# rsutormin/KmerGutsJava

Hardware: AMD Instinct MI355X
Metric: amino-acid residues/sec scanned (and hits/sec) on 1 Gbp synthetic, 1/2/4/8 MI355X (higher is better)
Workload: dtype int64; 1 GPU; 1 Gbp contig mix (0.5 kbp..1.024 Mbp, uniform ACGT) on 1 GPU, 6-frame translate + 8-mer lookup vs 1400303159-slot signature table (33.6 GB, load 0.50), -m 5 -g 200; total_bp_rank0=1000000000, contigs_rank0=6351, total_bp_all_ranks=1000000000, num_sigs=1400303159, residues_rank0=1999974596, residues_all_ranks=1999974596, hits_rank0=36744843, hits_all_ranks=36744843, calls_rank0=4, parallelism=contig shards x1, table replicated

## Files before the change

### kmergutsjava_amd/csrc/kg_host_plan.hpp

```cpp
#pragma once

namespace {


template <typename T, T V, T... Vs, typename F>
void dispatch(T x, F &&f)
{
    if constexpr (sizeof...(Vs) == 0) f(std::integral_constant<T, V>{});
    else if (x == V) f(std::integral_constant<T, V>{});
    else dispatch<T, Vs...>(x, f);
}

struct BatchPlan {
    std::vector<uint32_t> ibase;
    uint64_t nblocks = 0, windows = 0, residues = 0;
    uint64_t n_rows = 0, n_cont = 0;
    int64_t longest = 0;
};

template <bool AA>
int plan_batch(const int64_t *offsets, int64_t n_seqs, BatchPlan &b)
{
    constexpr uint32_t PER = AA ? 1 : 6;
    b.ibase.resize((size_t)n_seqs + 1);
    for (int64_t k = 0; k < n_seqs; k++) {
        int64_t L = offsets[k + 1] - offsets[k];
        if (L < 0) return fail(KG_ERR_ARG, "offsets must be non-decreasing");
        b.longest = std::max(b.longest, L);
        if (L > 0xFFFFFFF0ll) return fail(KG_ERR_LIMIT, "a single sequence longer than 2^32-16 characters");
        b.ibase[(size_t)k] = (uint32_t)b.nblocks;
        uint64_t nb;
        if (AA) {
            uint64_t nwin = L >= 9 ? (uint64_t)L - 8 : 0;
            b.windows += nwin;
            b.residues += (uint64_t)L;
            nb = (nwin + kg::kAaWinPerBlock - 1) / kg::kAaWinPerBlock;
        } else {
            uint64_t npos = L >= 24 ? (uint64_t)L - 23 : 0;
            b.windows += 2 * npos;
            for (int f = 0; f < 3; f++)
                if (L - f >= 3) b.residues += 2 * (uint64_t)((L - f) / 3);
            nb = (npos + kg::kDnaPosPerBlock - 1) / kg::kDnaPosPerBlock;
        }
        b.nblocks += nb;
        if (b.nblocks > 0x7FFFFFFFull / PER) return fail(KG_ERR_LIMIT, "batch too large: more than 2^31-1 window rows; split the batch");
    }
    b.ibase[(size_t)n_seqs] = (uint32_t)b.nblocks;
    if (b.windows > 0xFFFFFF00ull) return fail(KG_ERR_LIMIT, "batch too large: more than 2^32-256 windows; split the batch");
    b.n_rows = b.nblocks * PER;
    b.n_cont = (uint64_t)n_seqs * PER;
    return KG_OK;
}

uint64_t bucket_count(uint64_t limit, uint32_t shift) { return (limit + (1ull << shift) - 1) >> shift; }

struct PartPlan {
    bool applicable = false;
    uint32_t shift = 0, buckets = 0;
    uint32_t n_chunks = 0;
    std::vector<uint64_t> clo;
    std::vector<int64_t> cseq;
    uint64_t max_chunk = 0;
    uint32_t n_wg = 0, cap = 0;
    uint64_t n_regions = 0;
    uint32_t ovf_cap = 0;
    uint32_t gshift = 10, groups_stride = 0;
    size_t next_stride = 0;
    size_t scatter_lds = 0;
    bool use_bidx = false, part_counters = false, prog_index = false;
    uint32_t probe_grid = 0, index_grid = 0, verify_grid = 0, lowc_grid = 0, ovf_grid = 0, order_grid = 0;
    uint32_t scatter_prio = 0, index_prio = 0, verify_prio = 0, index_r = 1, probe_grab = 0;
    uint64_t list_slack = 0, ucap = 0, ccap = 0;
    uint32_t n_os = 0;
    bool early_totals = false, place_staged = false, debug = false;
};

template <bool AA>
int plan_partition(const kg_table *t, const BatchPlan &b, bool progress, bool counters_req, PartPlan &pl)
{
    constexpr uint32_t PER = AA ? 1 : 6;
    const uint64_t nblocks = b.nblocks;
    uint32_t shift = env_knob("KG_PART_SHIFT", 21u, 4u, 31u);
    const uint64_t qmax = (uint64_t)KG_MAX_ENCODED / (uint64_t)t->num_sigs + 1;
    while (shift > 4 && qmax >= (1ull << (32 - shift))) shift--;
    while (bucket_count(t->limit, shift) > (uint64_t)kg::kMaxBuckets) shift++;
    while (kg::scatter_lds_bytes<AA>((uint32_t)bucket_count(t->limit, shift)) > 160u * 1024) shift++;
    const bool fits = shift < 32 && qmax < (1ull << (32 - shift)) && nblocks <= (1ull << 23) && t->m35 != 0 &&
                      t->limit < (1ull << 32) - 64;
    const uint32_t mode = env_u32("KG_PARTITION", 2u);
    const bool worth = t->limit >= (64ull << 20) && b.windows >= (1ull << 27);
    if (!(fits && nblocks > 0 && (mode == 1 || (mode == 2 && worth)))) return KG_OK;
    pl.shift = shift;
    pl.buckets = (uint32_t)bucket_count(t->limit, shift);

    constexpr uint32_t WIN = AA ? 64u : 384u;
    uint32_t want = env_u32("KG_PART_CHUNKS", 4u);
    if (want < 1) want = 1;
    if (want > kMaxChunks) want = kMaxChunks;
    if (getenv("KG_PART_MIN_CHUNK_BLOCKS")) {
        const uint64_t min_chunk = std::max(1u, env_u32("KG_PART_MIN_CHUNK_BLOCKS", 600000u));
        while (want > 1 && nblocks / want < min_chunk) want--;
    } else {
        const uint32_t by_size = nblocks < 450000 ? 1u : std::max(2u, (uint32_t)std::lround(std::sqrt((double)nblocks / 325000.0)));
        want = std::min(want, std::max(1u, by_size));
    }
    pl.clo.push_back(0); pl.cseq.push_back(0);
    std::vector<double> cum;
    if (const char *tp = getenv("KG_PART_TAPER")) {
        double acc = 0;
        for (const char *q = tp; *q;) {
            char *endp = nullptr;
            const double v = strtod(q, &endp);
            if (endp == q) break;
            acc += v; cum.push_back(acc);
            q = *endp == ',' ? endp + 1 : endp;
        }
        if (cum.size() >= 2 && cum.size() <= kMaxChunks && acc > 0) { for (auto &x : cum) x /= acc; want = (uint32_t)cum.size(); }
        else cum.clear();
    }
    for (uint32_t c = 1; c < want; c++) {
        const uint64_t target = cum.empty() ? nblocks * c / want : (uint64_t)((double)nblocks * cum[c - 1]);
        const auto it = std::lower_bound(b.ibase.begin(), b.ibase.end(), (uint32_t)target);
        const uint64_t cut = *it;
        if (cut > pl.clo.back() && cut < nblocks) { pl.clo.push_back(cut); pl.cseq.push_back((int64_t)(it - b.ibase.begin())); }
    }
    pl.clo.push_back(nblocks); pl.cseq.push_back((int64_t)b.ibase.size() - 1);
    pl.n_chunks = (uint32_t)pl.clo.size() - 1;
    for (uint32_t c = 0; c < pl.n_chunks; c++) pl.max_chunk = std::max(pl.max_chunk, pl.clo[c + 1] - pl.clo[c]);
    const uint64_t max_chunk = pl.max_chunk;
    const uint64_t chunk_blocks = (max_chunk + kg::kScatterWaves - 1) / kg::kScatterWaves * kg::kScatterWaves;
    const double max_frac = (double)max_chunk / (double)nblocks;
    uint32_t n_wg = env_knob("KG_PART_WGS", 256u, 1u, kMaxGrid);
    if ((uint64_t)n_wg * kg::kScatterWaves > chunk_blocks) n_wg = (uint32_t)((chunk_blocks + kg::kScatterWaves - 1) / kg::kScatterWaves);
    const uint64_t blocks_per_wg = ((chunk_blocks + (uint64_t)n_wg * kg::kScatterWaves - 1) / ((uint64_t)n_wg * kg::kScatterWaves)) * kg::kScatterWaves;
    const double mean = (double)blocks_per_wg * WIN / (double)pl.buckets * (env_u32("KG_PART_SLACK", 100u) / 100.0);
    const uint64_t cap64 = ((uint64_t)(mean + 6.0 * std::sqrt(mean) + 32.0) + 15) / 16 * 16;
    if (cap64 >= (1ull << 24) || (uint64_t)pl.buckets * n_wg >= (1ull << 24)) return KG_OK;
    pl.n_wg = n_wg;
    pl.cap = (uint32_t)cap64;
    pl.n_regions = (uint64_t)pl.buckets * n_wg;
    pl.ovf_cap = env_u32("KG_PART_OVF_GROUPS", (uint32_t)std::min<uint64_t>(1u << 23, std::max<uint64_t>(65536, pl.n_regions * pl.cap / 16 / 8)));
    while (pl.gshift < 12 && ((max_chunk * PER) >> pl.gshift) + 2 > 8192) pl.gshift++;
    pl.groups_stride = (uint32_t)(((max_chunk * PER) >> pl.gshift) + 2);
    if (pl.groups_stride > kg::kMaxGroups) return fail(KG_ERR_LIMIT, "a chunk of the batch holds more than 2^26 window rows");
    pl.next_stride = std::max<size_t>((size_t)pl.buckets + 8, 256);
    pl.use_bidx = t->d_bidx != nullptr && !counters_req && env_u32("KG_BIDX", 1u) != 0;
    pl.part_counters = (counters_req || progress) && !pl.use_bidx;
    pl.prog_index = progress && pl.use_bidx;
    pl.scatter_lds = kg::scatter_lds_bytes<AA>(pl.buckets);
    pl.probe_grid = env_knob("KG_PROBE_GRID", 256u * 8u, 8u, kMaxGrid, 8u);
    pl.index_grid = env_knob("KG_INDEX_GRID", 256u * 4u, 8u, kMaxGrid, 8u);
    pl.scatter_prio = std::min(3u, env_u32("KG_SCATTER_PRIO", 1u));
    pl.index_prio = std::min(3u, env_u32("KG_INDEX_PRIO", 2u));
    pl.verify_prio = std::min(3u, env_u32("KG_VERIFY_PRIO", pl.n_chunks == 1 ? 2u : 0u));
    uint32_t index_r = env_u32("KG_INDEX_R", 0u);
    if (index_r == 0) index_r = mean * 0.7 >= 640.0 ? 1u : mean * 0.7 >= 320.0 ? 2u : 4u;
    if (index_r != 1 && index_r != 2) index_r = 4;
    while (index_r > 1 && (n_wg % index_r != 0 || kg::kIndexN % index_r != 0)) index_r /= 2;
    pl.index_r = index_r;
    pl.verify_grid = env_knob("KG_VERIFY_GRID", 256u * 2u, 1u, kMaxGrid);
    pl.lowc_grid = env_knob("KG_LOWC_GRID", 256u, 1u, kMaxGrid);
    pl.ovf_grid = env_knob("KG_OVF_GRID", 256u, 1u, kMaxGrid);
    pl.list_slack = (uint64_t)(std::max(std::max(pl.probe_grid, pl.index_grid), pl.verify_grid) + 64) * 4 * kg::kUChunk + 4096;
    pl.ucap = ((uint64_t)((double)b.windows * t->stage_ratio * max_frac) + pl.list_slack + kg::kUChunk - 1) / kg::kUChunk * kg::kUChunk;
    pl.ccap = ((uint64_t)((double)b.windows * (t->stage_ratio * 1.25 + 0.03) * max_frac) + pl.list_slack + kg::kUChunk - 1) /
              kg::kUChunk * kg::kUChunk;
    if (test_hook("KG_TEST_TINY_LISTS")) pl.ucap = pl.ccap = kg::kUChunk;
    const uint32_t grab_unit = 256u * (uint32_t)std::max(kg::kProbeN, kg::kIndexN);
    pl.probe_grab = env_knob("KG_PROBE_GRAB", pl.cap, grab_unit, 1u << 24, grab_unit);
    pl.n_os = pl.n_chunks < 2 ? 0u : std::min(env_u32("KG_ORDER_STREAMS", 0u), kMaxOrderStreams);
    pl.early_totals = pl.n_os == 0 && env_u32("KG_EARLY_TOTALS", 1u) != 0;
    pl.order_grid = env_knob("KG_ORDER_GRID", 256u * 3u, 1u, kMaxGrid);
    pl.place_staged = pl.gshift == 10 && env_u32("KG_PLACE_STAGED", 1u) != 0;
    pl.debug = getenv("KG_DEBUG") != nullptr;
    pl.applicable = true;
    return KG_OK;
}

struct DirectPlan {
    uint32_t scan_grid, stage_chunk;
    const uint32_t *d_hbits;
    uint32_t rpg;
    uint64_t stage_cap;
};

template <bool AA>
DirectPlan plan_direct(const kg_table *t, const BatchPlan &b, bool counters)
{
    DirectPlan pl;
    pl.scan_grid = env_knob("KG_SCAN_GRID", 256u * 8u, 1u, kMaxGrid);
    pl.stage_chunk = env_knob("KG_STAGE_CHUNK", 256u, 1u, 1u << 12);
    const uint32_t filter_mode = env_u32("KG_DIRECT_FILTER", 1u);
    pl.d_hbits = (counters || filter_mode == 0 || (filter_mode == 1 && t->limit <= (4ull << 20))) ? nullptr : t->d_hbits;
    pl.rpg = AA ? 1u : env_u32("KG_SCAN_RPG", pl.d_hbits ? 6u : 3u);
    if (pl.rpg != 1 && pl.rpg != 2 && pl.rpg != 3 && pl.rpg != 6) pl.rpg = 3;
    pl.stage_cap = (uint64_t)((double)b.windows * t->stage_ratio) + 4096 + (uint64_t)pl.scan_grid * kg::kWavesPerWG * pl.stage_chunk;
    if (pl.stage_cap > 0xFFFFFF00ull) pl.stage_cap = 0xFFFFFF00ull;
    if (test_hook("KG_TEST_TINY_LISTS")) pl.stage_cap = 256;
    return pl;
}

struct AggPlan {
    uint32_t pshift;
    bool pieces_on;
    uint32_t agg_pairs;
};

AggPlan plan_aggregate()
{
    AggPlan pl;
    pl.pshift = std::min(20u, std::max(6u, env_u32("KG_AGG_BLOCK_SHIFT", 9u)));
    pl.pieces_on = env_u32("KG_AGG_PIECES", 1u) != 0;
    pl.agg_pairs = env_u32("KG_AGG_PAIRS", 1u);
    return pl;
}

}
```

### kmergutsjava_amd/csrc/kg_host_scan.hpp

```cpp
#pragma once

namespace {

struct ScanCtx {
    kg_table *t;
    kg_result *res;
    Scratch &sc;
    const BatchPlan &b;
    const uint8_t *d_seq, *h_seq;
    const int64_t *offsets;
    int64_t n_seqs;
    bool progress, counters;
    bool seq_uploaded;
    uint64_t n_hits = 0;
    int64_t *d_off = nullptr;
    uint32_t *d_ibase = nullptr;
    kg::BlockDesc *d_blocks = nullptr;
    uint32_t *d_counts = nullptr, *d_offs = nullptr, *d_bsb = nullptr;
    uint64_t *d_partial = nullptr, *d_totals = nullptr;
    kg::Progress *d_prog = nullptr;
};

int upload_seq(const ScanCtx &cx, int64_t a, int64_t b)
{
// ... 114 lines not shown
    size_t cused_stride = 0, candused_stride = 0;
    kg_hit *d_ulist = nullptr, *d_sortA = nullptr, *d_sortB = nullptr;
    uint32_t *d_cused = nullptr, *d_candused = nullptr;
    kg::CandRec *d_cand = nullptr;
};

struct ChunkView {
    uint32_t c, lo, nb;
    uint64_t *ent, *ovf_ent;
    uint32_t *fill, *next, *ovfc, *ovf_bucket;
    kg_hit *ulist, *sortA, *sortB;
    uint32_t *cused, *candused;
    kg::CandRec *cand;
    unsigned long long *ucur, *ccur;
    uint64_t *base, *ctot;
    uint32_t *ghist, *gbase, *gcur1, *gcur2, *gtile;
};

ChunkView chunk_view(const PartPlan &pl, const PartBuffers &pb, uint32_t c)
{
    ChunkView v;
    v.c = c; v.lo = (uint32_t)pl.clo[c]; v.nb = (uint32_t)(pl.clo[c + 1] - pl.clo[c]);
    v.ent = pb.d_ent + (uint64_t)c * pl.n_regions * pl.cap;
    v.fill = pb.d_fill + (uint64_t)c * pl.n_regions;
    v.next = pb.d_next + (size_t)c * pl.next_stride;
    v.ovfc = pb.d_ovfc + kOvfWords * c; v.ovf_bucket = pb.d_ovf_bucket + (size_t)c * pl.ovf_cap;
    v.ovf_ent = pb.d_ovf_ent + (size_t)c * pl.ovf_cap * kg::kGroup;
    v.ulist = pb.d_ulist + (uint64_t)c * pb.ucap;
    v.cused = pb.d_cused + c * pb.cused_stride; v.candused = pb.d_candused + c * pb.candused_stride;
    v.cand = pb.d_cand + (uint64_t)c * pb.ccap;
    v.ucur = (unsigned long long *)(pb.d_pc + kPcUcur + c); v.ccur = (unsigned long long *)(pb.d_pc + kPcCcur + c);
    v.base = pb.d_pc + kPcBase + c; v.ctot = pb.d_pc + kPcCtot + c;
    v.ghist = pb.d_ghist + (size_t)c * pl.groups_stride; v.gbase = pb.d_gbase + (size_t)c * (pl.groups_stride + 1);
    v.gcur1 = pb.d_gcur1 + (size_t)c * (kg::kHDigits + 1); v.gcur2 = pb.d_gcur2 + (size_t)c * pl.groups_stride;
    v.gtile = pb.d_gtile + (size_t)c * (kg::kHDigits + 1);
    v.sortA = pb.d_sortA + (uint64_t)c * pb.ucap; v.sortB = pb.d_sortB + (uint64_t)c * pb.ucap;
    return v;
}

int scatter_variant_of(const ScanCtx &cx)
{
    return cx.t->limit >= (uint64_t)cx.t->num_sigs ? 0 : cx.d_prog ? 2 : 1;
}
template <typename F>
void scatter_variant(int variant, F &&f)
{
    if (variant == 0) f(std::false_type{}, std::false_type{});
    else if (variant == 1) f(std::true_type{}, std::false_type{});
    else f(std::true_type{}, std::true_type{});
}

int upload_scatter_cold(const ScanCtx &cx, const PartPlan &pl, const PartBuffers &pb)
{
    kg_table *t = cx.t;
    kg::ScatterCold h[kMaxChunks] = {};
    for (uint32_t c = 0; c < pl.n_chunks; c++) {
        uint32_t *ovfc = pb.d_ovfc + kOvfWords * c;
        h[c].ovf_cursor = ovfc; h[c].ovf_bucket = pb.d_ovf_bucket + (size_t)c * pl.ovf_cap;
        h[c].ovf_ent = pb.d_ovf_ent + (size_t)c * pl.ovf_cap * kg::kGroup;
        h[c].lowc_cursor = ovfc + kOvfLowc; h[c].lowc_blocks = pb.d_lowc + pl.clo[c];
        h[c].ctr = (unsigned long long *)(cx.d_totals + kTotValid); h[c].prog = cx.d_prog;
        h[c].ovf_cap = pl.ovf_cap;
    }
    if (!t->d_cold) HIP_TRY(hipMalloc((void **)&t->d_cold, sizeof h));
    else if (!memcmp(h, t->h_cold, sizeof h)) return KG_OK;
    memcpy(t->h_cold, h, sizeof h);
    HIP_TRY(hipMemcpyAsync(t->d_cold, t->h_cold, sizeof h, hipMemcpyHostToDevice, t->stream));
    return KG_OK;
}

template <bool AA>
int chunk_passes(const ScanCtx &cx, const PartPlan &pl, const PartBuffers &pb, const ChunkView &v)
{
    kg_table *t = cx.t;
    kg::Progress *d_prog = cx.d_prog;
    unsigned long long *d_ctr = (unsigned long long *)(cx.d_totals + kTotValid);
    const hipStream_t s2 = t->stream2, s3 = t->stream3;
    uint32_t *lowc_cursor = v.ovfc + kOvfLowc, *lowc = pb.d_lowc + v.lo;
    const uint32_t limit32 = (uint32_t)std::min<uint64_t>(t->limit, 0xFFFFFFFFull);
    scatter_variant(scatter_variant_of(cx), [&](auto is_short, auto prog) {
        constexpr bool SHORT = decltype(is_short)::value, PROG = decltype(prog)::value;
        hipLaunchKernelGGL((kg::part_scatter_kernel<AA, SHORT, PROG>), dim3(pl.n_wg), dim3(kg::kWave * kg::kScatterWaves), pl.scatter_lds,
                           t->stream, cx.d_seq, cx.d_blocks, v.lo, v.nb, limit32, (uint32_t)t->num_sigs, t->m35, pl.shift, pl.buckets, pl.cap,
                           v.ent, v.fill, t->d_cold + v.c, pl.scatter_prio);
    });
    HIP_TRY(hipEventRecord(t->pev[kPevChunk + 2 * v.c], t->stream));
    HIP_TRY(hipStreamWaitEvent(s2, t->pev[kPevChunk + 2 * v.c], 0));
    hipLaunchKernelGGL((kg::lowc_blocks_kernel<AA>), dim3(pl.lowc_grid), dim3(64 * kg::kLowcWaves), 0, s2, cx.d_seq, cx.d_blocks, lowc_cursor, lowc,
                       t->limit, (uint32_t)t->num_sigs, t->m35, pl.shift, pl.n_wg, pl.cap, v.ent, v.fill, v.ovfc, pl.ovf_cap,
                       v.ovf_bucket, v.ovf_ent, d_ctr, d_prog);
    if (pl.use_bidx) {
        const uint32_t tail_start = (uint32_t)std::min<uint64_t>(t->tail_start, 0xFFFFFFFFull);
        dispatch<int, 1, 2, 4>((int)pl.index_r, [&](auto r) {
            dispatch<bool, true, false>(t->bidx_exact, [&](auto exact) {
                dispatch<bool, true, false>(pl.prog_index, [&](auto prog) {
                    constexpr int R = decltype(r)::value;
                    constexpr bool EXACT = decltype(exact)::value, PROG = decltype(prog)::value;
                    hipLaunchKernelGGL((kg::bucket_index_kernel<kg::kIndexN, R, EXACT, PROG>), dim3(pl.index_grid), dim3(256), 0, s2,
                                       t->d_bidx, tail_start, v.ent, v.fill, pl.n_wg, pl.cap, pl.buckets, pl.shift, pl.probe_grab, v.next,
                                       v.cand, v.candused, v.ccur, pb.ccap, d_ctr, pl.index_prio, PROG ? d_prog : (kg::Progress *)nullptr);
                });
            });
        });
    } else {
        dispatch<bool, true, false>(pl.part_counters, [&](auto counters) {
            constexpr bool COUNTERS = decltype(counters)::value;
            hipLaunchKernelGGL((kg::bucket_tag_kernel<COUNTERS>), dim3(pl.probe_grid), dim3(256), 0, s2, t->d_tags, t->limit,
                               (uint64_t)t->num_sigs, v.ent, v.fill, pl.n_wg, pl.cap, pl.buckets, pl.shift, pl.probe_grab, v.next, v.cand,
                               v.candused, v.ccur, pb.ccap, d_ctr, COUNTERS ? d_prog : (kg::Progress *)nullptr);
        });
    }
    HIP_TRY(hipEventRecord(t->pev[kPevChunk + 2 * v.c + 1], s2));
    HIP_TRY(hipStreamWaitEvent(s3, t->pev[kPevChunk + 2 * v.c + 1], 0));
    dispatch<int, 1, 2, 0>(pl.part_counters ? 1 : pl.prog_index ? 2 : 0, [&](auto walks) {
        constexpr bool COUNTERS = decltype(walks)::value == 1, PROG = decltype(walks)::value == 2;
        hipLaunchKernelGGL((kg::verify_kernel<AA, COUNTERS, PROG>), dim3(pl.verify_grid), dim3(256), 0, s3, t->d_entries, t->d_tags, t->limit,
                           (uint64_t)t->num_sigs, t->magic, v.cand, v.candused, v.ccur, pb.ccap, v.ulist, v.cused, v.ucur, pb.ucap, d_ctr,
                           d_prog, pl.verify_prio);
        hipLaunchKernelGGL((kg::overflow_probe_kernel<AA, COUNTERS, PROG>), dim3(pl.ovf_grid), dim3(256), 0, s3, t->d_entries, t->d_tags,
                           t->limit, (uint64_t)t->num_sigs, t->magic, v.ovf_bucket, v.ovf_ent, v.ovfc, pl.ovf_cap, pl.shift, v.ulist,
                           v.cused, v.ucur, pb.ucap, d_ctr, d_prog);
    });
    HIP_TRY(hipEventRecord(t->pev[kPevVerified + v.c], s3));
    HIP_TRY(hipGetLastError());
    return KG_OK;
}

template <bool AA>
int chunk_order(const ScanCtx &cx, const PartPlan &pl, const PartBuffers &pb, const ChunkView &v, uint64_t hits_cap)
{
    constexpr uint32_t PER = AA ? 1 : 6;
    kg_table *t = cx.t;
    kg_result *res = cx.res;
    const uint32_t c = v.c, gshift = pl.gshift;
    const bool last = c + 1 == pl.n_chunks;
    hipStream_t s = t->stream;
    if (pl.n_os) {
        s = t->ostream[c % pl.n_os];
        HIP_TRY(hipStreamWaitEvent(s, t->ev[kEvScattered], 0));
    }
    HIP_TRY(hipStreamWaitEvent(s, t->pev[kPevVerified + c], 0));
    const uint64_t row_lo = (uint64_t)v.lo * PER, row_hi = row_lo + (uint64_t)v.nb * PER;
    const uint32_t g0 = (uint32_t)(row_lo >> gshift);
    const uint32_t n_groups = v.nb ? (uint32_t)(((row_hi - 1) >> gshift) - g0 + 1) : 1u;
    hipLaunchKernelGGL(kg::hit_hist_kernel, dim3(pl.order_grid), dim3(kg::kHThreads), (size_t)n_groups * 4, s, v.ulist, v.cused, v.ucur, pb.ucap,
                       g0, 6u + gshift, n_groups, v.ghist);
    hipLaunchKernelGGL(kg::group_scan_kernel, dim3(1), dim3(kg::kGsThreads), 0, s, v.ghist, n_groups, v.gbase, v.gcur1, v.gcur2, v.ctot, v.gtile);
    if (pl.n_os && c) HIP_TRY(hipStreamWaitEvent(s, t->pev[kPevBase + c - 1], 0));
    hipLaunchKernelGGL(kg::chunk_base_kernel, dim3(1), dim3(1), 0, s, v.ctot, v.base, last ? cx.d_totals : (uint64_t *)nullptr);
    if (pl.n_os) HIP_TRY(hipEventRecord(t->pev[kPevBase + c], s));
    if (pl.early_totals && last) {
        int rc;
        if ((rc = send_counters(t, pb.d_pc, pb.d_ovfc, cx.d_totals, s))) return rc;
        HIP_TRY(hipEventRecord(t->pev[kPevTotals], s));
    }
    hipLaunchKernelGGL((kg::hit_partition_kernel<true>), dim3(pl.order_grid), dim3(kg::kHThreads), 0, s, v.ulist, v.cused, v.ucur, pb.ucap,
                       v.gbase, n_groups, g0, 6u + gshift, v.gcur1, v.sortA, pb.ucap, v.gtile);
    hipLaunchKernelGGL((kg::hit_partition_kernel<false>), dim3(pl.order_grid), dim3(kg::kHThreads), 0, s, v.sortA, v.cused, v.ucur, pb.ucap,
                       v.gbase, n_groups, g0, 6u + gshift, v.gcur2, v.sortB, pb.ucap, v.gtile);
    hipLaunchKernelGGL((kg::group_place_kernel<AA>), dim3(std::min(n_groups, 256u * 8u)), dim3(kg::kHThreads),
                       kg::group_place_lds(gshift, pl.place_staged), s,
                       v.sortB, v.gbase, n_groups, g0, gshift, (uint32_t)row_lo, (uint32_t)row_hi, pb.d_geo, (uint64_t)cx.b.n_rows,
                       pl.place_staged ? 1u : 0u, v.base, res->d_hits, hits_cap, cx.d_offs, res->d_hit_slots);
    HIP_TRY(hipGetLastError());
    return KG_OK;
}

// ... 346 lines not shown
```

### kmergutsjava_amd/csrc/kg_partition.hpp

```cpp
#pragma once

#include "kg_device.hpp"

namespace kg {

constexpr int kMaxBuckets = 1024;
#ifndef KG_PROBE_N
#define KG_PROBE_N 4
#endif
#ifndef KG_SCATTER_WPE
#define KG_SCATTER_WPE 5
#endif
#ifndef KG_TAG_WPE
#define KG_TAG_WPE 8
#endif
#if KG_SCATTER_WPE
#define KG_SCATTER_REGS __attribute__((amdgpu_waves_per_eu(KG_SCATTER_WPE)))
#else
#define KG_SCATTER_REGS
#endif
#if KG_TAG_WPE
#define KG_TAG_REGS __attribute__((amdgpu_waves_per_eu(KG_TAG_WPE)))
#else
#define KG_TAG_REGS
#endif
#ifndef KG_STAGE_FLUSH
#define KG_STAGE_FLUSH 64
#endif
#ifndef KG_SCATTER_RG
#define KG_SCATTER_RG 6
#endif

#ifndef KG_SCAN_FULL
#define KG_SCAN_FULL 1
#endif

constexpr uint32_t kStageFlush = KG_STAGE_FLUSH;
constexpr int kProbeN = KG_PROBE_N;
#ifndef KG_INDEX_N
#define KG_INDEX_N KG_PROBE_N
#endif
constexpr int kIndexN = KG_INDEX_N;
constexpr uint32_t kUChunk = 512;

constexpr uint64_t kEntInvalid = ~0ull;

template <bool AA>
__device__ __forceinline__ uint32_t window_key(const BlockDesc &bd, uint32_t it, int r, int lane)
{
    const uint32_t ol = (!AA && r >= 3) ? 63u - (uint32_t)lane : (uint32_t)lane;
    return (row_index<AA>(bd, it, r) << 6) | ol;
}
#ifndef KG_SCATTER_WAVES
#define KG_SCATTER_WAVES 16
#endif
constexpr int kScatterWaves = KG_SCATTER_WAVES;
constexpr uint32_t kGroup = 16;

template <bool AA>
inline size_t scatter_lds_bytes(uint32_t n_buckets)
{
    size_t enc = (sizeof(typename WaveLds<AA>::type) + 15) & ~(size_t)15;
    size_t tab = (sizeof(typename WaveLds<AA>::tables) + 15) & ~(size_t)15;
    return enc * kScatterWaves + tab + (size_t)n_buckets * (kGroup * 8 + 12);
}

#ifndef KG_SCATTER_NT
#define KG_SCATTER_NT 1
#endif
__device__ __forceinline__ void store_entry_pair(uint64_t *dst, const ulonglong2 &v)
{
#if KG_SCATTER_NT
    typedef uint64_t u64x2 __attribute__((ext_vector_type(2)));
    u64x2 x; x.x = v.x; x.y = v.y;
    __builtin_nontemporal_store(x, reinterpret_cast<u64x2 *>(dst));
#else
    *reinterpret_cast<ulonglong2 *>(dst) = v;
#endif
}

struct ScatterCold {
    uint32_t *ovf_cursor;
    uint32_t *ovf_bucket;
    uint64_t *ovf_ent;
    uint32_t *lowc_cursor;
    uint32_t *lowc_blocks;
    unsigned long long *ctr;
    Progress *prog;
    uint32_t ovf_cap, pad;
};
static_assert(sizeof(ScatterCold) == 64, "ScatterCold is one 64-byte line");

constexpr unsigned long long kDstOvf = 1ull << 62, kDstNone = ~0ull, kDstDropped = ~0ull - 1;

__device__ __attribute__((noinline, cold)) unsigned long long scatter_overflow_groups(const ScatterCold *__restrict__ cold,
                                                                                     unsigned long long movf, bool to_ovf, uint32_t b,
                                                                                     unsigned long long dst)
{
    const int lane = threadIdx.x & 63;
    uint32_t og = 0;
    if (lane == 0) og = atomicAdd(cold->ovf_cursor, (uint32_t)__popcll(movf));
    og = (uint32_t)__builtin_amdgcn_readfirstlane((int)og);
    if (to_ovf) {
        const uint32_t g = og + (uint32_t)__popcll(movf & ((1ull << lane) - 1ull));
        if (g < cold->ovf_cap) { cold->ovf_bucket[g] = b; dst = kDstOvf | ((uint64_t)g * kGroup); }
        else dst = kDstDropped;
    }
    return dst;
}
__device__ __attribute__((noinline, cold)) void scatter_set_aside(const ScatterCold *__restrict__ cold, uint32_t block)
{
    if ((threadIdx.x & 63) == 0) cold->lowc_blocks[atomicAdd(cold->lowc_cursor, 1u)] = block;
}
__device__ __attribute__((noinline, cold)) void scatter_protocol_failure(const ScatterCold *__restrict__ cold)
{
    if ((threadIdx.x & 63) == 0) atomicOr(cold->ovf_cursor + 2, 1u);
}
__device__ __forceinline__ void store_group_part(uint64_t *__restrict__ ent, const ScatterCold *__restrict__ cold, unsigned long long to,
                                                 uint32_t sub, const ulonglong2 &v)
{
    if (__builtin_expect((to & kDstOvf) != 0, 0)) store_entry_pair(cold->ovf_ent + (to & ~kDstOvf) + 2 * sub, v);
    else store_entry_pair(ent + to + 2 * sub, v);
}
__device__ __attribute__((noinline, cold)) void scatter_note_beyond(const ScatterCold *__restrict__ cold, uint32_t slot)
{
    progress_note_beyond(cold->prog, slot);
}

struct BlockRows { uint32_t len, j, nk, ibase; };
__device__ __forceinline__ BlockRows rows_of(const BlockDesc &bd) { return BlockRows{bd.len, bd.j, bd.nk, bd.ibase}; }
__device__ __forceinline__ BlockDesc desc_of(const BlockRows &r)
{
    BlockDesc bd;
    bd.soff = 0; bd.len = r.len; bd.j = r.j; bd.nk = r.nk; bd.ibase = r.ibase; bd.seq = 0; bd.pad = 0;
    return bd;
}

template <bool AA, bool SHORT = false, bool PROG = false>
__global__ __launch_bounds__(kWave *kScatterWaves) KG_SCATTER_REGS void part_scatter_kernel(
    const uint8_t *__restrict__ seq, const BlockDesc *__restrict__ blocks, uint32_t block_lo, uint32_t n_blocks ,
    uint32_t limit32 , uint32_t num_sigs , uint32_t m35, uint32_t shift,
    uint32_t n_buckets, uint32_t cap, uint64_t *__restrict__ ent, uint32_t *__restrict__ fill, const ScatterCold *__restrict__ cold,
    uint32_t insert_prio )
{
    static_assert(SHORT || !PROG, "PROG implies SHORT");
    constexpr int ROWS = AA ? 1 : 6;
    typedef typename WaveLds<AA>::type Enc;
    constexpr size_t enc_bytes = (sizeof(Enc) + 15) & ~(size_t)15;
    extern __shared__ __attribute__((aligned(16))) unsigned char part_lds[];
    const int lane = threadIdx.x & 63, wave = __builtin_amdgcn_readfirstlane((int)(threadIdx.x >> 6));
    Enc &l = *reinterpret_cast<Enc *>(part_lds + enc_bytes * wave);
    typedef typename WaveLds<AA>::tables Tables;
    constexpr size_t tab_bytes = (sizeof(Tables) + 15) & ~(size_t)15;
    Tables &enc_tables = *reinterpret_cast<Tables *>(part_lds + enc_bytes * kScatterWaves);
    uint64_t *buf = reinterpret_cast<uint64_t *>(part_lds + enc_bytes * kScatterWaves + tab_bytes);
    uint32_t *cnt = reinterpret_cast<uint32_t *>(buf + (size_t)n_buckets * kGroup);
    uint32_t *wrel = cnt + n_buckets;
    uint32_t *written = wrel + n_buckets;
    const uint32_t w = blockIdx.x, n_wg = gridDim.x;
    for (uint32_t b = threadIdx.x; b < n_buckets; b += blockDim.x) { cnt[b] = 0; wrel[b] = 0; written[b] = 0; }
    encode_init<AA>(enc_tables, threadIdx.x, blockDim.x);
    __syncthreads();

    uint32_t n_valid = 0;
    bool ran_off = false;
    const uint32_t n_iter = (n_blocks + n_wg * kScatterWaves - 1) / (n_wg * kScatterWaves);
    BlockRows rows_next = {0, 0, 0, 0};
    uint32_t raw_next[4] = {0, 0, 0, 0};
    {
        const uint32_t it0 = w * kScatterWaves + (uint32_t)wave;
        if (it0 < n_blocks) {
            const BlockDesc bd0 = blocks[block_lo + it0];
            load_block_chars<AA>(seq, bd0, lane, raw_next);
            rows_next = rows_of(bd0);
        }
    }
    constexpr int RG = AA ? 1 : KG_SCATTER_RG;
    static_assert(ROWS % RG == 0, "KG_SCATTER_RG must divide 6");
    for (uint32_t iter = 0; iter < n_iter; iter++) {
        const uint32_t it = (iter * n_wg + w) * kScatterWaves + (uint32_t)wave;
        const BlockDesc bd = desc_of(rows_next);
        const bool have = it < n_blocks;
        if (have) {
            uint32_t raw[4] = {raw_next[0], raw_next[1], raw_next[2], raw_next[3]};
            const uint32_t itn = it + n_wg * kScatterWaves;
            if (itn < n_blocks) {
                const BlockDesc bdn = blocks[block_lo + itn];
                load_block_chars<AA>(seq, bdn, lane, raw_next);
                rows_next = rows_of(bdn);
            }
            encode_chars<AA>(l, enc_tables, raw, lane);
        }
        bool lowc = false;
#pragma unroll
        for (int g0 = 0; g0 < ROWS; g0 += RG) {
        uint64_t e[RG];
        uint32_t bk[RG];
        uint32_t pend = 0, nv = 0;
        if (have && !lowc) {
#pragma unroll
            for (int k = 0; k < RG; k++) {
                const int r = g0 + k;
                uint32_t hi, lo, q;
                bool valid = row_halves<AA>(l, r, lane, bd, &hi, &lo);
                const uint32_t slot = split_fast(hi, lo, num_sigs, m35, &q);
                if (valid) nv++;
                if constexpr (SHORT) {
                    if (valid && slot >= limit32) {
                        ran_off = true;
                        if constexpr (PROG) scatter_note_beyond(cold, slot);
                    }
                    valid = valid && slot < limit32;
                }
                bk[k] = slot >> shift;
                const uint32_t low = (q << shift) | (slot & ((1u << shift) - 1u));
                const uint32_t id = window_key<AA>(bd, block_lo + it, r, lane);
                e[k] = ((uint64_t)id << 32) | low;
                if (valid) pend |= 1u << k;
            }
            if (g0 + RG == ROWS) wave_sync();
            if (g0 == 0) {
                const unsigned long long m0 = __ballot((pend & 1u) != 0);
                if (__popcll(m0) >= 32) {
                    const uint32_t lead0 = (uint32_t)__builtin_amdgcn_readlane((int)bk[0], __builtin_ctzll(m0));
                    if (__builtin_expect(__popcll(__ballot((pend & 1u) && bk[0] == lead0)) >= 24, 0)) {
                        scatter_set_aside(cold, block_lo + it);
                        nv = 0;
                        pend = 0;
                        lowc = true;
                        if (RG != ROWS) wave_sync();
                    }
                }
            }
        }
        n_valid += nv;
        uint32_t done = 0, spins = 0;
        if (insert_prio) set_wave_prio(insert_prio);
        for (;;) {
            uint32_t at[RG];
#pragma unroll
            for (int r = 0; r < RG; r++)
                at[r] = (pend & (1u << r)) ? atomicAdd(&cnt[bk[r]], 1u) : kGroup;
#pragma unroll
            for (int r = 0; r < RG; r++)
                if (at[r] < kGroup) buf[(size_t)bk[r] * kGroup + at[r]] = e[r];
            __builtin_amdgcn_fence(__ATOMIC_RELEASE, "workgroup");
#pragma unroll
            for (int r = 0; r < RG; r++)
                if (at[r] < kGroup) {
                    pend &= ~(1u << r);
                    if (atomicAdd(&written[bk[r]], 1u) == kGroup - 1) done |= 1u << r;
                }
            __builtin_amdgcn_fence(__ATOMIC_ACQUIRE, "workgroup");
            for (;;) {
                const bool has = done != 0;
                unsigned long long m = __ballot(has);
                if (!m) break;
                const int r0 = has ? __builtin_ctz(done) : 0;
                uint32_t b = bk[0];
#pragma unroll
                for (int r = 1; r < RG; r++)
                    if (r0 == r) b = bk[r];
                unsigned long long dst = kDstNone;
                bool to_ovf = false;
                if (has) {
                    done &= done - 1;
                    const uint32_t rel = wrel[b];
                    if (rel + kGroup <= cap) {
                        dst = mul24_wide(b * n_wg + w, cap) + rel;
                        wrel[b] = rel + kGroup;
                    } else {
                        to_ovf = true;
                    }
                }
                const unsigned long long movf = __ballot(to_ovf);
                if (__builtin_expect(movf != 0, 0)) dst = scatter_overflow_groups(cold, movf, to_ovf, b, dst);
                uint8_t *rank_lane = reinterpret_cast<uint8_t *>(&l);
                const uint32_t n_flush = (uint32_t)__popcll(m);
                if (has) rank_lane[__popcll(m & ((1ull << lane) - 1ull))] = (uint8_t)lane;
                wave_sync();
                for (uint32_t p0 = 0; p0 < n_flush; p0 += 8) {
                    const uint32_t want = p0 + ((uint32_t)lane >> 3);
                    const bool serve = want < n_flush;
                    const int sl = serve ? (int)rank_lane[want] : 0;
                    const uint32_t fb = (uint32_t)__shfl((int)b, sl);
                    const unsigned long long to = __shfl(dst, sl);
                    if (serve && to != kDstDropped) {
                        const uint32_t sub = (uint32_t)lane & 7u;
                        const ulonglong2 v = *reinterpret_cast<const ulonglong2 *>(buf + (size_t)fb * kGroup + 2 * sub);
                        store_group_part(ent, cold, to, sub, v);
                    }
                }
                wave_sync();
                if (has) { written[b] = 0; __builtin_amdgcn_fence(__ATOMIC_RELEASE, "workgroup"); cnt[b] = 0; }
            }
            if (!__ballot(pend != 0)) break;
            {
                const int rp = pend ? __builtin_ctz(pend) : 0;
                uint32_t pb = bk[0];
#pragma unroll
                for (int r = 1; r < RG; r++)
                    if (rp == r) pb = bk[r];
                for (uint32_t polls = 0; polls < 64; polls++) {
                    if (__ballot(pend != 0 && __hip_atomic_load(&cnt[pb], __ATOMIC_RELAXED, __HIP_MEMORY_SCOPE_WORKGROUP) < kGroup)) break;
                    __builtin_amdgcn_s_sleep(2);
                }
            }
            uint32_t at_max = at[0];
#pragma unroll
            for (int r = 1; r < RG; r++) at_max = max(at_max, at[r]);
            if (__builtin_expect(++spins > (1u << 20) || __ballot(at_max >= (1u << 28)), 0)) {
                scatter_protocol_failure(cold);
                break;
            }
        }
        if (insert_prio) set_wave_prio(0);
        }
    }
    __syncthreads();
    const uint32_t per_wave = (n_buckets + kScatterWaves - 1) / kScatterWaves;
    const uint32_t b_end = min((uint32_t)(wave + 1) * per_wave, n_buckets);
    for (uint32_t b0 = (uint32_t)wave * per_wave; b0 < b_end; b0 += 64) {
        const uint32_t b = b0 + (uint32_t)lane;
        const uint32_t c = b < b_end ? cnt[b] : 0u;
        unsigned long long dst = kDstNone;
        bool to_ovf = false;
        if (c > 0) {
            for (uint32_t k = c; k < kGroup; k++) buf[(size_t)b * kGroup + k] = kEntInvalid;
            const uint32_t rel = wrel[b];
            if (rel + kGroup <= cap) {
                dst = ((uint64_t)b * n_wg + w) * cap + rel;
                wrel[b] = rel + kGroup;
            } else {
                to_ovf = true;
            }
            cnt[b] = 0;
        }
        const unsigned long long movf = __ballot(to_ovf);
        if (movf) dst = scatter_overflow_groups(cold, movf, to_ovf, b, dst);
        unsigned long long m = __ballot(dst != kDstNone);
        wave_sync();
        while (m) {
            int src_lane = -1;
            unsigned long long mm = m;
#pragma unroll
            for (int g = 0; g < 8; g++) {
                const int ln = mm ? __builtin_ctzll(mm) : -1;
                if (mm) mm &= mm - 1;
                if ((lane >> 3) == g) src_lane = ln;
            }
            m = mm;
            const int sl = src_lane < 0 ? 0 : src_lane;
            const uint32_t fb = (uint32_t)__shfl((int)b, sl);
            const unsigned long long to = __shfl(dst, sl);
            if (src_lane >= 0 && to != kDstDropped) {
                const uint32_t sub = (uint32_t)lane & 7u;
                const ulonglong2 v = *reinterpret_cast<const ulonglong2 *>(buf + (size_t)fb * kGroup + 2 * sub);
                store_group_part(ent, cold, to, sub, v);
            }
        }
    }
    __syncthreads();
    for (uint32_t b = threadIdx.x; b < n_buckets; b += blockDim.x) fill[(uint64_t)b * n_wg + w] = wrel[b];
    for (int off = 32; off > 0; off >>= 1) n_valid += __shfl_down(n_valid, off);
    unsigned long long *ctr = cold->ctr;
    if (lane == 0 && n_valid) atomicAdd(&ctr[0], (unsigned long long)n_valid);
    if constexpr (SHORT) flush_ran_off(ran_off, ctr, lane);
}

constexpr int kLowcWaves = 4;
template <bool AA>
__global__ __launch_bounds__(64 * kLowcWaves) void lowc_blocks_kernel(
    const uint8_t *__restrict__ seq, const BlockDesc *__restrict__ blocks, const uint32_t *__restrict__ lowc_cursor,
    const uint32_t *__restrict__ lowc_blocks, uint64_t limit, uint32_t num_sigs, uint32_t m35, uint32_t shift, uint32_t n_regions,
    uint32_t cap, uint64_t *__restrict__ ent, uint32_t *__restrict__ fill, uint32_t *ovf_cursor, uint32_t ovf_cap,
    uint32_t *__restrict__ ovf_bucket, uint64_t *__restrict__ ovf_ent, unsigned long long *ctr, Progress *prog)
{
    constexpr int ROWS = AA ? 1 : 6;
    __shared__ typename WaveLds<AA>::type lds[kLowcWaves];
    __shared__ typename WaveLds<AA>::tables enc_tables;
    const int lane = threadIdx.x & 63, wave = threadIdx.x >> 6;
    typename WaveLds<AA>::type &l = lds[wave];
    const uint32_t n_list = *lowc_cursor;
    if (n_list == 0) return;
    encode_init<AA>(enc_tables, threadIdx.x, blockDim.x);
    __syncthreads();
    const uint32_t limit32 = limit < 0xFFFFFFFFull ? (uint32_t)limit : 0xFFFFFFFFu;
    unsigned long long n_valid = 0;
    bool ran_off = false;
    uint32_t pool_at = 0, pool_end = 0;
    auto pool_flush = [&]() {
        for (uint32_t g = pool_at + ((uint32_t)lane >> 4); g < pool_end && g < ovf_cap; g += 4) {
            if ((lane & 15) == 0) ovf_bucket[g] = 0;
            ovf_ent[(uint64_t)g * kGroup + ((uint32_t)lane & 15u)] = kEntInvalid;
        }
        pool_at = pool_end;
    };
    auto ovf_groups = [&](uint32_t lead, uint32_t ng) -> uint64_t * {
        if (pool_end - pool_at < ng) {
            pool_flush();
            const uint32_t want = ng > 32u ? ng : 32u;
            uint32_t g0 = 0;
            if (lane == 0) g0 = atomicAdd(ovf_cursor, want);
            g0 = (uint32_t)__builtin_amdgcn_readfirstlane((int)g0);
            pool_at = g0; pool_end = g0 + want;
        }
        const uint32_t g = pool_at;
        pool_at += ng;
        if (g + ng > ovf_cap) return nullptr;
        if ((uint32_t)lane < ng) ovf_bucket[g + lane] = lead;
        return ovf_ent + (uint64_t)g * kGroup;
    };
    for (uint32_t i = blockIdx.x * kLowcWaves + (uint32_t)wave; i < n_list; i += gridDim.x * kLowcWaves) {
        const uint32_t it = (uint32_t)__builtin_amdgcn_readfirstlane((int)lowc_blocks[i]);
        const BlockDesc bd = blocks[it];
        encode_block<AA>(l, enc_tables, seq, bd, lane);
        const uint32_t region_w = it % n_regions;
        for (int r = 0; r < ROWS; r++) {
            uint32_t hi, lo, q;
            bool valid = row_halves<AA>(l, r, lane, bd, &hi, &lo);
            const uint32_t slot = split_fast(hi, lo, num_sigs, m35, &q);
            if (valid) n_valid++;
            if (valid && slot >= limit32) { ran_off = true; if (prog) progress_note_beyond(prog, slot); }
            bool pend = valid && slot < limit32;
            const uint32_t bkt = slot >> shift;
            const uint64_t e = ((uint64_t)window_key<AA>(bd, it, r, lane) << 32) | ((q << shift) | (slot & ((1u << shift) - 1u)));
            for (int pass = 0; pass < 4; pass++) {
                const unsigned long long mp = __ballot(pend);
                if (__popcll(mp) < 16) break;
                const uint32_t lead = (uint32_t)__builtin_amdgcn_readlane((int)bkt, __builtin_ctzll(mp));
                const bool mine = pend && bkt == lead;
                const unsigned long long same = __ballot(mine);
                const uint32_t n = (uint32_t)__popcll(same);
                if (n < 8) break;
                const uint32_t rank = (uint32_t)__popcll(same & ((1ull << lane) - 1ull));
                const uint64_t region = (uint64_t)lead * n_regions + region_w;
                uint32_t rel = cap;
                if (lane == 0 && *const_cast<volatile uint32_t *>(&fill[region]) < cap) rel = atomicAdd(&fill[region], n);
                rel = (uint32_t)__builtin_amdgcn_readfirstlane((int)rel);
                if (rel + n <= cap) {
                    if (mine) ent[region * cap + rel + rank] = e;
                } else {
                    if (rel < cap && (uint32_t)lane < cap - rel) ent[region * cap + rel + lane] = kEntInvalid;
                    const uint32_t npad = (n + kGroup - 1) & ~(kGroup - 1);
                    uint64_t *dst = ovf_groups(lead, npad / kGroup);
                    if (dst) {
// ... 554 lines not shown
```

Measured before the change: 129.0 billion residues/s.

## Derive scatter group slot from written counter and flush via per-wave list

The scatter kernel no longer keeps a per-bucket write cursor (wrel). The group index is taken from a running `written` counter, so the lane that completes a 16-entry group knows its output offset directly. Full groups are recorded in a per-wave LDS flush list and stored by 8-lane octets, with workgroup fences relaxed to wavefront scope. Overflow handling moves into cold noinline helpers. This removes one LDS array, the per-flush ballot/rank loop and the wrel read-modify-write, but it makes the concurrency protocol more subtle (cnt reset ordering, fill computed from written).

```diff
diff --git a/kmergutsjava_amd/csrc/kg_host_plan.hpp b/kmergutsjava_amd/csrc/kg_host_plan.hpp
--- a/kmergutsjava_amd/csrc/kg_host_plan.hpp
+++ b/kmergutsjava_amd/csrc/kg_host_plan.hpp
@@ -70,6 +70,7 @@
     bool use_bidx = false, part_counters = false, prog_index = false;
     uint32_t probe_grid = 0, index_grid = 0, verify_grid = 0, lowc_grid = 0, ovf_grid = 0, order_grid = 0;
     uint32_t scatter_prio = 0, index_prio = 0, verify_prio = 0, index_r = 1, probe_grab = 0;
+    uint32_t flush_list = 0;
     uint64_t list_slack = 0, ucap = 0, ccap = 0;
     uint32_t n_os = 0;
     bool early_totals = false, place_staged = false, debug = false;
@@ -148,6 +149,7 @@
     pl.part_counters = (counters_req || progress) && !pl.use_bidx;
     pl.prog_index = progress && pl.use_bidx;
     pl.scatter_lds = kg::scatter_lds_bytes<AA>(pl.buckets);
+    pl.flush_list = env_knob("KG_SCATTER_FLUSH_LIST", kg::scatter_flush_list_max<AA>(), 1u, kg::scatter_flush_list_max<AA>());
     pl.probe_grid = env_knob("KG_PROBE_GRID", 256u * 8u, 8u, kMaxGrid, 8u);
     pl.index_grid = env_knob("KG_INDEX_GRID", 256u * 4u, 8u, kMaxGrid, 8u);
     pl.scatter_prio = std::min(3u, env_u32("KG_SCATTER_PRIO", 1u));
diff --git a/kmergutsjava_amd/csrc/kg_host_scan.hpp b/kmergutsjava_amd/csrc/kg_host_scan.hpp
--- a/kmergutsjava_amd/csrc/kg_host_scan.hpp
+++ b/kmergutsjava_amd/csrc/kg_host_scan.hpp
@@ -220,7 +220,7 @@
         constexpr bool SHORT = decltype(is_short)::value, PROG = decltype(prog)::value;
         hipLaunchKernelGGL((kg::part_scatter_kernel<AA, SHORT, PROG>), dim3(pl.n_wg), dim3(kg::kWave * kg::kScatterWaves), pl.scatter_lds,
                            t->stream, cx.d_seq, cx.d_blocks, v.lo, v.nb, limit32, (uint32_t)t->num_sigs, t->m35, pl.shift, pl.buckets, pl.cap,
-                           v.ent, v.fill, t->d_cold + v.c, pl.scatter_prio);
+                           v.ent, v.fill, t->d_cold + v.c, pl.scatter_prio, pl.flush_list);
     });
     HIP_TRY(hipEventRecord(t->pev[kPevChunk + 2 * v.c], t->stream));
     HIP_TRY(hipStreamWaitEvent(s2, t->pev[kPevChunk + 2 * v.c], 0));
diff --git a/kmergutsjava_amd/csrc/kg_partition.hpp b/kmergutsjava_amd/csrc/kg_partition.hpp
--- a/kmergutsjava_amd/csrc/kg_partition.hpp
+++ b/kmergutsjava_amd/csrc/kg_partition.hpp
@@ -62,7 +62,13 @@
 {
     size_t enc = (sizeof(typename WaveLds<AA>::type) + 15) & ~(size_t)15;
     size_t tab = (sizeof(typename WaveLds<AA>::tables) + 15) & ~(size_t)15;
-    return enc * kScatterWaves + tab + (size_t)n_buckets * (kGroup * 8 + 12);
+    return enc * kScatterWaves + tab + (size_t)n_buckets * (kGroup * 8 + 8);
+}
+template <bool AA>
+constexpr uint32_t scatter_flush_list_max()
+{
+    constexpr size_t idle = AA ? sizeof(WaveLdsAa) : KG_SCATTER_RG == 6 ? sizeof(WaveLdsDna) : sizeof(WaveLdsDna::bc);
+    return idle / 4 < 64 ? (uint32_t)(idle / 4) : 64u;
 }
 
 #ifndef KG_SCATTER_NT
@@ -93,9 +99,8 @@
 
 constexpr unsigned long long kDstOvf = 1ull << 62, kDstNone = ~0ull, kDstDropped = ~0ull - 1;
 
-__device__ __attribute__((noinline, cold)) unsigned long long scatter_overflow_groups(const ScatterCold *__restrict__ cold,
-                                                                                     unsigned long long movf, bool to_ovf, uint32_t b,
-                                                                                     unsigned long long dst)
+__device__ __forceinline__ unsigned long long overflow_reserve(const ScatterCold *__restrict__ cold, unsigned long long movf, bool to_ovf,
+                                                               uint32_t b, unsigned long long dst)
 {
     const int lane = threadIdx.x & 63;
     uint32_t og = 0;
@@ -108,6 +113,30 @@
     }
     return dst;
 }
+__device__ __attribute__((noinline, cold)) unsigned long long scatter_overflow_groups(const ScatterCold *__restrict__ cold,
+                                                                                     unsigned long long movf, bool to_ovf, uint32_t b,
+                                                                                     unsigned long long dst)
+{
+    return overflow_reserve(cold, movf, to_ovf, b, dst);
+}
+__device__ __attribute__((noinline, cold)) void scatter_overflow_octets(const ScatterCold *__restrict__ cold, bool full, uint32_t b,
+                                                                        uint64_t lo, uint64_t hi)
+{
+    const int lane = threadIdx.x & 63;
+    const bool lead = full && (lane & 7) == 0;
+    unsigned long long dst = overflow_reserve(cold, __ballot(lead), lead, b, kDstNone);
+    dst = __shfl(dst, lane & ~7);
+    if (full && dst != kDstDropped) {
+        ulonglong2 v; v.x = lo; v.y = hi;
+        store_entry_pair(cold->ovf_ent + (dst & ~kDstOvf) + 2 * ((uint32_t)lane & 7u), v);
+    }
+}
+__device__ __attribute__((noinline, cold)) void scatter_store_overflow(const ScatterCold *__restrict__ cold, unsigned long long to,
+                                                                       uint32_t sub, uint64_t lo, uint64_t hi)
+{
+    ulonglong2 v; v.x = lo; v.y = hi;
+    store_entry_pair(cold->ovf_ent + (to & ~kDstOvf) + 2 * sub, v);
+}
 __device__ __attribute__((noinline, cold)) void scatter_set_aside(const ScatterCold *__restrict__ cold, uint32_t block)
 {
     if ((threadIdx.x & 63) == 0) cold->lowc_blocks[atomicAdd(cold->lowc_cursor, 1u)] = block;
@@ -115,12 +144,6 @@
 __device__ __attribute__((noinline, cold)) void scatter_protocol_failure(const ScatterCold *__restrict__ cold)
 {
     if ((threadIdx.x & 63) == 0) atomicOr(cold->ovf_cursor + 2, 1u);
-}
-__device__ __forceinline__ void store_group_part(uint64_t *__restrict__ ent, const ScatterCold *__restrict__ cold, unsigned long long to,
-                                                 uint32_t sub, const ulonglong2 &v)
-{
-    if (__builtin_expect((to & kDstOvf) != 0, 0)) store_entry_pair(cold->ovf_ent + (to & ~kDstOvf) + 2 * sub, v);
-    else store_entry_pair(ent + to + 2 * sub, v);
 }
 __device__ __attribute__((noinline, cold)) void scatter_note_beyond(const ScatterCold *__restrict__ cold, uint32_t slot)
 {
@@ -141,7 +164,7 @@
     const uint8_t *__restrict__ seq, const BlockDesc *__restrict__ blocks, uint32_t block_lo, uint32_t n_blocks ,
     uint32_t limit32 , uint32_t num_sigs , uint32_t m35, uint32_t shift,
     uint32_t n_buckets, uint32_t cap, uint64_t *__restrict__ ent, uint32_t *__restrict__ fill, const ScatterCold *__restrict__ cold,
-    uint32_t insert_prio )
+    uint32_t insert_prio , uint32_t flush_list )
 {
     static_assert(SHORT || !PROG, "PROG implies SHORT");
     constexpr int ROWS = AA ? 1 : 6;
@@ -155,10 +178,12 @@
     Tables &enc_tables = *reinterpret_cast<Tables *>(part_lds + enc_bytes * kScatterWaves);
     uint64_t *buf = reinterpret_cast<uint64_t *>(part_lds + enc_bytes * kScatterWaves + tab_bytes);
     uint32_t *cnt = reinterpret_cast<uint32_t *>(buf + (size_t)n_buckets * kGroup);
-    uint32_t *wrel = cnt + n_buckets;
-    uint32_t *written = wrel + n_buckets;
+    uint32_t *written = cnt + n_buckets;
+    uint32_t *flist = reinterpret_cast<uint32_t *>(&l);
     const uint32_t w = blockIdx.x, n_wg = gridDim.x;
-    for (uint32_t b = threadIdx.x; b < n_buckets; b += blockDim.x) { cnt[b] = 0; wrel[b] = 0; written[b] = 0; }
+    const uint32_t gcap = cap >> 4;
+    const uint32_t list_cap = max(min(flush_list, scatter_flush_list_max<AA>()), 1u);
+    for (uint32_t b = threadIdx.x; b < n_buckets; b += blockDim.x) { cnt[b] = 0; written[b] = 0; }
     encode_init<AA>(enc_tables, threadIdx.x, blockDim.x);
     __syncthreads();
 
@@ -234,65 +259,81 @@
             }
         }
         n_valid += nv;
-        uint32_t done = 0, spins = 0;
+        uint32_t spins = 0;
         if (insert_prio) set_wave_prio(insert_prio);
         for (;;) {
-            uint32_t at[RG];
+            uint32_t at[RG], old[RG];
 #pragma unroll
             for (int r = 0; r < RG; r++)
                 at[r] = (pend & (1u << r)) ? atomicAdd(&cnt[bk[r]], 1u) : kGroup;
 #pragma unroll
-            for (int r = 0; r < RG; r++)
-                if (at[r] < kGroup) buf[(size_t)bk[r] * kGroup + at[r]] = e[r];
-            __builtin_amdgcn_fence(__ATOMIC_RELEASE, "workgroup");
-#pragma unroll
-            for (int r = 0; r < RG; r++)
+            for (int r = 0; r < RG; r++) {
+                old[r] = 0;
                 if (at[r] < kGroup) {
-                    pend &= ~(1u << r);
-                    if (atomicAdd(&written[bk[r]], 1u) == kGroup - 1) done |= 1u << r;
-                }
-            __builtin_amdgcn_fence(__ATOMIC_ACQUIRE, "workgroup");
-            for (;;) {
-                const bool has = done != 0;
-                unsigned long long m = __ballot(has);
-                if (!m) break;
-                const int r0 = has ? __builtin_ctz(done) : 0;
-                uint32_t b = bk[0];
-#pragma unroll
-                for (int r = 1; r < RG; r++)
-                    if (r0 == r) b = bk[r];
-                unsigned long long dst = kDstNone;
-                bool to_ovf = false;
-                if (has) {
-                    done &= done - 1;
-                    const uint32_t rel = wrel[b];
-                    if (rel + kGroup <= cap) {
-                        dst = mul24_wide(b * n_wg + w, cap) + rel;
-                        wrel[b] = rel + kGroup;
-                    } else {
-                        to_ovf = true;
-                    }
-                }
-                const unsigned long long movf = __ballot(to_ovf);
-                if (__builtin_expect(movf != 0, 0)) dst = scatter_overflow_groups(cold, movf, to_ovf, b, dst);
-                uint8_t *rank_lane = reinterpret_cast<uint8_t *>(&l);
-                const uint32_t n_flush = (uint32_t)__popcll(m);
-                if (has) rank_lane[__popcll(m & ((1ull << lane) - 1ull))] = (uint8_t)lane;
+                    buf[(size_t)bk[r] * kGroup + at[r]] = e[r];
+                    __builtin_amdgcn_fence(__ATOMIC_RELEASE, "wavefront");
+                    old[r] = atomicAdd(&written[bk[r]], 1u);
+                }
+            }
+            __builtin_amdgcn_fence(__ATOMIC_ACQUIRE, "wavefront");
+#pragma unroll
+            for (int r = 0; r < RG; r++) pend &= ~((uint32_t)(at[r] < kGroup) << r);
+            uint32_t at_max = at[0];
+#pragma unroll
+            for (int r = 1; r < RG; r++) at_max = max(at_max, at[r]);
+            uint32_t left = 0;
+            auto list_rows = [&](auto again) -> uint32_t {
+                uint32_t n = 0;
+#pragma unroll
+                for (int r = 0; r < RG; r++) {
+                    const bool own = decltype(again)::value ? ((left >> r) & 1u) != 0 : (old[r] & 15u) == 15u;
+                    const unsigned long long m = __ballot(own);
+                    if (m) {
+                        const uint32_t rank = __builtin_amdgcn_mbcnt_hi((uint32_t)(m >> 32), __builtin_amdgcn_mbcnt_lo((uint32_t)m, n));
+                        if (own && rank < list_cap) {
+                            const uint32_t g = decltype(again)::value ? (written[bk[r]] >> 4) - 1u : old[r] >> 4;
+                            flist[rank] = (min(g, gcap) << 10) | bk[r];
+                            if (decltype(again)::value) left &= ~(1u << r);
+                        }
+                        n += (uint32_t)__popcll(m);
+                    }
+                }
+                return n;
+            };
+            uint32_t n_own = list_rows(std::false_type{});
+            if (__builtin_expect(n_own > list_cap, 0)) {
+                uint32_t k = 0;
+#pragma unroll
+                for (int r = 0; r < RG; r++) {
+                    const bool own = (old[r] & 15u) == 15u;
+                    const unsigned long long m = __ballot(own);
+                    const uint32_t rank = __builtin_amdgcn_mbcnt_hi((uint32_t)(m >> 32), __builtin_amdgcn_mbcnt_lo((uint32_t)m, k));
+                    if (own && rank >= list_cap) left |= 1u << r;
+                    k += (uint32_t)__popcll(m);
+                }
+            }
+            while (n_own) {
+                const uint32_t n_list = min(n_own, list_cap);
                 wave_sync();
-                for (uint32_t p0 = 0; p0 < n_flush; p0 += 8) {
-                    const uint32_t want = p0 + ((uint32_t)lane >> 3);
-                    const bool serve = want < n_flush;
-                    const int sl = serve ? (int)rank_lane[want] : 0;
-                    const uint32_t fb = (uint32_t)__shfl((int)b, sl);
-                    const unsigned long long to = __shfl(dst, sl);
-                    if (serve && to != kDstDropped) {
-                        const uint32_t sub = (uint32_t)lane & 7u;
+                for (uint32_t p0 = 0; p0 < n_list; p0 += 8) {
+                    const uint32_t want = p0 + ((uint32_t)lane >> 3), sub = (uint32_t)lane & 7u;
+                    if (want < n_list) {
+                        const uint32_t d = flist[want];
+                        const uint32_t fb = d & (uint32_t)(kMaxBuckets - 1), g = d >> 10;
                         const ulonglong2 v = *reinterpret_cast<const ulonglong2 *>(buf + (size_t)fb * kGroup + 2 * sub);
-                        store_group_part(ent, cold, to, sub, v);
+                        __builtin_amdgcn_fence(__ATOMIC_RELEASE, "wavefront");
+                        if (sub == 0) cnt[fb] = 0;
+                        const bool full = g >= gcap;
+                        if (!full) {
+                            unsigned char *to = reinterpret_cast<unsigned char *>(ent) + (mul24_wide(__umul24(fb, n_wg) + w, cap) << 3);
+                            store_entry_pair(reinterpret_cast<uint64_t *>(to + ((g << 7) | (sub << 4))), v);
+                        }
+                        if (__builtin_expect(__ballot(full) != 0, 0)) scatter_overflow_octets(cold, full, fb, v.x, v.y);
                     }
                 }
                 wave_sync();
-                if (has) { written[b] = 0; __builtin_amdgcn_fence(__ATOMIC_RELEASE, "workgroup"); cnt[b] = 0; }
+                if (__builtin_expect(n_own <= list_cap, 1)) break;
+                n_own = list_rows(std::true_type{});
             }
             if (!__ballot(pend != 0)) break;
             {
@@ -306,9 +347,6 @@
                     __builtin_amdgcn_s_sleep(2);
                 }
             }
-            uint32_t at_max = at[0];
-#pragma unroll
-            for (int r = 1; r < RG; r++) at_max = max(at_max, at[r]);
             if (__builtin_expect(++spins > (1u << 20) || __ballot(at_max >= (1u << 28)), 0)) {
                 scatter_protocol_failure(cold);
                 break;
@@ -322,19 +360,14 @@
     const uint32_t b_end = min((uint32_t)(wave + 1) * per_wave, n_buckets);
     for (uint32_t b0 = (uint32_t)wave * per_wave; b0 < b_end; b0 += 64) {
         const uint32_t b = b0 + (uint32_t)lane;
-        const uint32_t c = b < b_end ? cnt[b] : 0u;
+        const uint32_t wr = b < b_end ? written[b] : 0u;
+        const uint32_t c = wr & 15u, g = wr >> 4;
         unsigned long long dst = kDstNone;
         bool to_ovf = false;
         if (c > 0) {
             for (uint32_t k = c; k < kGroup; k++) buf[(size_t)b * kGroup + k] = kEntInvalid;
-            const uint32_t rel = wrel[b];
-            if (rel + kGroup <= cap) {
-                dst = ((uint64_t)b * n_wg + w) * cap + rel;
-                wrel[b] = rel + kGroup;
-            } else {
-                to_ovf = true;
-            }
-            cnt[b] = 0;
+            if (g < gcap) dst = ((uint64_t)b * n_wg + w) * cap + ((uint64_t)g << 4);
+            else to_ovf = true;
         }
         const unsigned long long movf = __ballot(to_ovf);
         if (movf) dst = scatter_overflow_groups(cold, movf, to_ovf, b, dst);
@@ -344,24 +377,28 @@
             int src_lane = -1;
             unsigned long long mm = m;
 #pragma unroll
-            for (int g = 0; g < 8; g++) {
+            for (int o = 0; o < 8; o++) {
                 const int ln = mm ? __builtin_ctzll(mm) : -1;
                 if (mm) mm &= mm - 1;
-                if ((lane >> 3) == g) src_lane = ln;
+                if ((lane >> 3) == o) src_lane = ln;
             }
             m = mm;
             const int sl = src_lane < 0 ? 0 : src_lane;
             const uint32_t fb = (uint32_t)__shfl((int)b, sl);
             const unsigned long long to = __shfl(dst, sl);
-            if (src_lane >= 0 && to != kDstDropped) {
+            if (src_lane >= 0) {
                 const uint32_t sub = (uint32_t)lane & 7u;
                 const ulonglong2 v = *reinterpret_cast<const ulonglong2 *>(buf + (size_t)fb * kGroup + 2 * sub);
-                store_group_part(ent, cold, to, sub, v);
-            }
-        }
-    }
-    __syncthreads();
-    for (uint32_t b = threadIdx.x; b < n_buckets; b += blockDim.x) fill[(uint64_t)b * n_wg + w] = wrel[b];
+                if (__builtin_expect((to & kDstOvf) != 0, 0)) {
+                    if (to != kDstDropped) scatter_store_overflow(cold, to, sub, v.x, v.y);
+                } else {
+                    store_entry_pair(ent + to + 2 * sub, v);
+                }
+            }
+        }
+    }
+    for (uint32_t b = threadIdx.x; b < n_buckets; b += blockDim.x)
+        fill[(uint64_t)b * n_wg + w] = min((written[b] + 15u) >> 4, gcap) << 4;
     for (int off = 32; off > 0; off >>= 1) n_valid += __shfl_down(n_valid, off);
     unsigned long long *ctr = cold->ctr;
     if (lane == 0 && n_valid) atomicAdd(&ctr[0], (unsigned long long)n_valid);
```

Measured after the change: 131.9 billion residues/s, median of 6. 2.3% higher.
